# thomasjungblut/go-sstables

Hardware: AMD Instinct MI355X
Metric: recordio decode GiB/s (device-resident), v4 1 KiB records, 1/2/4/8 GPU (higher is better)
Workload: dtype u8; 1 GPU; C2: recordio v4, 1M x 1 KiB snappy records (text-like), one file per GPU; records=1000000, record_bytes=1024, decoded_bytes=1024000000, compression=snappy, parallelism=file-sharded x1 (1 files), no data-path collectives

## Files before the change

go-sstables_amd/csrc/rio_ctx.cpp:

```cpp
#include <algorithm>
#include <cstring>
#include <iterator>
#include <map>

#include "rio_ctx.h"
#include "rio_host.h"

using namespace rio;

extern "C" const char* rio_strerror(int s) {
    switch (s) {
    case RIO_OK: return "ok";
    case RIO_EOF: return "EOF";
    case RIO_EOF_ZERO_TAIL: return "EOF (zero-padded tail)";
    case RIO_EOF_HEADER: return "EOF inside record header";
    case RIO_EOF_PAYLOAD: return "EOF reading record payload";
    case RIO_ERR_UNEXPECTED_EOF: return "unexpected EOF";
    case RIO_ERR_MAGIC: return "magic number mismatch";
    case RIO_ERR_HEADER_CRC: return "header checksum mismatch";
    case RIO_ERR_VARINT_OVERFLOW: return "binary: varint overflows a 64-bit integer";
    case RIO_ERR_HEADER_TOO_LONG: return "checksum byte reader out of range";
    case RIO_ERR_DECOMPRESS: return "snappy: corrupt input";
    case RIO_ERR_VERSION: return "version mismatch";
    case RIO_ERR_COMPRESSION_TYPE: return "unknown compression type";
    case RIO_ERR_SHORT_FILE_HEADER: return "not enough bytes in the file header";
    case RIO_ERR_INVALID_OFFSET: return "mmap: invalid ReadAt offset";
    case RIO_ERR_UNSUPPORTED: return "not supported by the GPU decode path";
    case RIO_ERR_CAPACITY: return "output capacity too small";
    case RIO_ERR_ARG: return "invalid argument";
    case RIO_ERR_HIP: return "HIP runtime error";
    case RIO_ERR_STATE: return "reader state error";
    case RIO_ERR_IO: return "I/O error";
    case RIO_ERR_PROTO: return "proto: cannot parse invalid wire-format data";
    case RIO_EOF_CODEC: return "EOF from the codec (empty gzip payload)";
    default: return "unknown status";
    }
}

extern "C" int rio_status_is_eof(int s) {
    return s == RIO_EOF || s == RIO_EOF_ZERO_TAIL || s == RIO_EOF_HEADER || s == RIO_EOF_PAYLOAD || s == RIO_EOF_CODEC;
}

extern "C" const char* rio_build_info(void) { return "librio gfx950 recordio v3/v4 decode"; }

extern "C" uint64_t rio_max_records(uint64_t len) {
    return len <= RIO_FILE_HEADER_BYTES ? 1 : (len - RIO_FILE_HEADER_BYTES) / 5 + 1;
}

constexpr uint64_t kLaneWalkMin = 768, kLaneWalkMax = 8192, kLaneWalkChunks = 32768;
constexpr uint64_t kLaneWalkSmallMin = 512, kLaneWalkSmallChunks = 65536;
constexpr uint64_t kBigRecordChunk = 65536;
constexpr uint64_t kSmallFileChunkMin = 8192, kWalkWavesPerSimd = 5;
static uint64_t wave_chunk_bytes(const rio_ctx* ctx, uint64_t len) {
    const uint64_t cb = ctx->fr.chunk_bytes;
    if (!ctx->fr.chunk_auto) return cb;
    const uint64_t slots = ctx->fr.walk_slots;
    const uint64_t want = ((len + slots - 1) / slots + 4095) & ~4095ull;
    return std::min(cb, std::max(want, kSmallFileChunkMin));
}

struct ArenaSizes {
    uint64_t n_chunks, slots, n_blocks, scratch, meta;
};
static ArenaSizes arena_sizes(uint64_t len, uint64_t cb) {
    ArenaSizes z;
    z.n_chunks = len > RIO_FILE_HEADER_BYTES ? (len - RIO_FILE_HEADER_BYTES + cb - 1) / cb : 0;
    z.slots = cb / 5 + 1;
    z.n_blocks = (z.n_chunks + 255) / 256;
    const uint64_t nc = std::max<uint64_t>(z.n_chunks, 1), nb = std::max<uint64_t>(z.n_blocks, 1);
    z.scratch = nc * z.slots * 8;
    auto al = [](uint64_t x) { return (x + 255) & ~255ull; };
    z.meta = al(sizeof(ScanState)) + al(sizeof(rio_file_info)) + 2 * al(nb * sizeof(RunSum)) +
             al(2 * kFailLanes * sizeof(uint64_t)) + al(nc * sizeof(ChunkSum)) + al(nc * sizeof(RunSum)) +
             al(nc * sizeof(ChunkPlace));
    return z;
}

int rio::ctx_frame_params(rio_ctx* ctx, const uint8_t* d_file, uint64_t len, FrameParams& P, FileArenas& A,
                          bool reserve_all) {
    const rio_ctx::Framing& F = ctx->fr;
    memset(&P, 0, sizeof P);
    P.file = d_file;
    P.len = len;
    bool lane = F.walk_mode == 1;
    if (F.walk_mode == 2 && F.walk_hint && len / F.lane_chunk_bytes >= kLaneWalkChunks) {
        const uint64_t m = *reinterpret_cast<volatile uint64_t*>(F.walk_hint);
        const uint64_t chunks = len / F.lane_chunk_bytes;
        lane = (m >= kLaneWalkMin && m <= kLaneWalkMax) ||
               (m >= F.lane_walk_min && m < kLaneWalkMin && chunks >= kLaneWalkSmallChunks);
    }
    uint64_t cb = lane ? F.lane_chunk_bytes : wave_chunk_bytes(ctx, len);
    if (!lane && F.chunk_auto && F.walk_hint && *reinterpret_cast<volatile uint64_t*>(F.walk_hint) > kLaneWalkMax)
        cb = std::max<uint64_t>(cb, kBigRecordChunk);
    P.walk_lane = lane ? 1u : 0u;
    P.walk_hint = F.walk_hint;
    P.chunk_bytes = cb;
    P.coop_min = F.coop_min;
    P.comp_hint = RIO_COMP_UNKNOWN;
    P.zero_done = 0;
    const ArenaSizes z = arena_sizes(len, cb);
    P.n_chunks = z.n_chunks;
    P.slots = z.slots;
    P.n_blocks = z.n_blocks;
    const uint64_t nc = std::max<uint64_t>(P.n_chunks, 1), nb = std::max<uint64_t>(P.n_blocks, 1);
    uint64_t scr = z.scratch, meta_need = z.meta;
    if (reserve_all) {
        for (uint64_t c : {wave_chunk_bytes(ctx, len), F.chunk_bytes, F.lane_chunk_bytes,
                           std::max<uint64_t>(F.chunk_bytes, kBigRecordChunk)}) {
            const ArenaSizes y = arena_sizes(len, c);
            scr = std::max(scr, y.scratch);
            meta_need = std::max(meta_need, y.meta);
        }
    }
    HIP_TRY(A.scratch_off.ensure(scr));
    HIP_TRY(A.scratch_len.ensure(scr));
    HIP_TRY(A.scratch_pay.ensure(scr));
    auto al = [](uint64_t x) { return (x + 255) & ~255ull; };
    const uint64_t o_info = al(sizeof(ScanState)), o_brun = o_info + al(sizeof(rio_file_info));
    const uint64_t o_bexc = o_brun + al(nb * sizeof(RunSum)), o_fail = o_bexc + al(nb * sizeof(RunSum));
    const uint64_t o_chk = o_fail + al(2 * kFailLanes * sizeof(uint64_t)), o_cexc = o_chk + al(nc * sizeof(ChunkSum));
    const uint64_t o_place = o_cexc + al(nc * sizeof(RunSum)), meta_bytes = o_place + al(nc * sizeof(ChunkPlace));
    HIP_TRY(A.meta.ensure(std::max(meta_bytes, meta_need)));
    HIP_TRY(ctx->fr.sink.ensure(kSinkBytes));
    uint8_t* const mb = A.meta.as<uint8_t>();
    P.sink = F.sink.as<uint8_t>();
    P.fail_lanes = reinterpret_cast<uint64_t*>(mb + o_fail);
    P.scratch_off = A.scratch_off.as<uint64_t>();
    P.scratch_len = A.scratch_len.as<uint64_t>();
    P.scratch_pay = A.scratch_pay.as<uint64_t>();
    P.chunks = reinterpret_cast<ChunkSum*>(mb + o_chk);
    P.chunk_excl = reinterpret_cast<RunSum*>(mb + o_cexc);
    P.place = reinterpret_cast<ChunkPlace*>(mb + o_place);
    P.block_runs = reinterpret_cast<RunSum*>(mb + o_brun);
    P.block_excl = reinterpret_cast<RunSum*>(mb + o_bexc);
    P.state = reinterpret_cast<ScanState*>(mb);
    P.info = reinterpret_cast<rio_file_info*>(mb + o_info);
    return RIO_OK;
}

extern "C" int rio_device_count(int* out) {
    int n = 0;
    if (hipGetDeviceCount(&n) != hipSuccess) n = 0;
    if (out) *out = n;
    return n > 0 ? RIO_OK : RIO_ERR_HIP;
}

extern "C" int rio_ctx_create(int device, rio_ctx** out) {
    if (!out) return RIO_ERR_ARG;
    *out = nullptr;
    int n = 0;
    if (hipGetDeviceCount(&n) != hipSuccess || n <= 0) return RIO_ERR_HIP;
    if (device < 0 || device >= n) return RIO_ERR_ARG;
    HIP_TRY(hipSetDevice(device));
    auto* c = new rio_ctx();
    rio_ctx::Framing& F = c->fr;
    c->device = device;
    F.chunk_bytes = env_u64("RIO_CHUNK_BYTES", 32768);
    F.chunk_auto = std::getenv("RIO_CHUNK_BYTES") == nullptr;
    if (F.chunk_bytes < 64 || F.chunk_bytes > (1ull << 30) || (F.chunk_bytes & 15)) F.chunk_bytes = 32768;
    F.walk_mode = (uint32_t)std::min<uint64_t>(env_u64("RIO_WALK_LANE", 2), 2);
    F.lane_chunk_bytes = env_u64("RIO_LANE_CHUNK_BYTES", 16384);
    F.lane_walk_min = env_u64("RIO_LANE_WALK_MIN", kLaneWalkSmallMin);
    int cus = 0;
    if (hipDeviceGetAttribute(&cus, hipDeviceAttributeMultiprocessorCount, device) == hipSuccess && cus > 0)
        F.walk_slots = (uint64_t)cus * 4 * kWalkWavesPerSimd;
    if (F.lane_chunk_bytes < 64 || F.lane_chunk_bytes > (1ull << 30) || (F.lane_chunk_bytes & 15))
        F.lane_chunk_bytes = 16384;
    if (hipHostMalloc(reinterpret_cast<void**>(&F.walk_hint), sizeof(uint64_t), hipHostMallocPortable) != hipSuccess) {
        (void)hipGetLastError();
        F.walk_hint = nullptr;
    } else {
        *F.walk_hint = 0;
    }
    F.coop_min = env_u64("RIO_COOP_MIN", ~0ull >> 8);
    if (hipStreamCreateWithFlags(&c->stream, hipStreamNonBlocking) != hipSuccess) {
        delete c;
        return RIO_ERR_HIP;
    }
    c->timing.set_ring(0);
    *out = c;
    return RIO_OK;
}

extern "C" int rio_ctx_device(const rio_ctx* c) { return c ? c->device : -1; }

extern "C" void rio_ctx_destroy(rio_ctx* c) {
    if (!c) return;
    hipSetDevice(c->device);
    hipStreamSynchronize(c->stream);
    if (c->order.ev) hipEventSynchronize(c->order.ev);
    c->mrg.views.wait();
    c->wal.segs.wait();
    delete c;
}

extern "C" int rio_ctx_set_timing(rio_ctx* c, int slots) {
    if (!c || slots < 0) return RIO_ERR_ARG;
    hipSetDevice(c->device);
    hipStreamSynchronize(c->stream);
// ... 191 lines not shown
```

go-sstables_amd/csrc/rio_ctx.h:

```cpp
#pragma once
#include <hip/hip_runtime.h>

#include <algorithm>
#include <array>
#include <cstdlib>
#include <memory>
#include <mutex>
#include <vector>

#include "rio_host.h"
#include "rio_launch.h"

#define HIP_TRY(x)                                  \
    do {                                            \
        hipError_t e_ = (x);                        \
        if (e_ != hipSuccess) return RIO_ERR_HIP;   \
    } while (0)

namespace rio {

inline int hip_status(hipError_t e) { return e == hipSuccess ? RIO_OK : RIO_ERR_HIP; }

inline bool header_refused(int s) {
    return s == RIO_ERR_VERSION || s == RIO_ERR_COMPRESSION_TYPE || s == RIO_ERR_SHORT_FILE_HEADER;
// ... 1 lines not shown
inline bool nothing_framed(int s) { return header_refused(s) || s == RIO_ERR_UNSUPPORTED; }

inline uint64_t env_u64(const char* name, uint64_t dflt) {
    const char* v = getenv(name);
    if (!v || !*v) return dflt;
    return strtoull(v, nullptr, 0);
}

struct DevBuf {
    void* p = nullptr;
    size_t cap = 0;
    DevBuf() = default;
    DevBuf(const DevBuf&) = delete;
    DevBuf& operator=(const DevBuf&) = delete;
    ~DevBuf() { release(); }
    hipError_t ensure(size_t n) {
        if (n <= cap) return hipSuccess;
        release();
        size_t want = std::max<size_t>(n, 256);
        hipError_t e = hipMalloc(&p, want);
        if (e == hipSuccess) cap = want;
        return e;
    }
    void release() {
        if (p) hipFree(p);
        p = nullptr;
        cap = 0;
    }
    template <class T>
    T* as() const { return static_cast<T*>(p); }
};

struct FileArenas {
    DevBuf scratch_off, scratch_len, scratch_pay, rec_pay, rec_desc, meta;
    uint64_t bytes() const {
        return scratch_off.cap + scratch_len.cap + scratch_pay.cap + rec_pay.cap + rec_desc.cap + meta.cap;
    }
};

struct PlanUpload {
    DevBuf dev;
    std::vector<uint64_t> host;
    hipEvent_t ev = nullptr;
    ~PlanUpload() {
        wait();
        if (ev) hipEventDestroy(ev);
    }
    hipError_t upload(std::vector<uint64_t>& fresh, hipStream_t s) {
        hipError_t e = ev ? hipEventSynchronize(ev) : hipEventCreateWithFlags(&ev, hipEventDisableTiming);
        if (e != hipSuccess) return e;
        host.swap(fresh);
        e = hipMemcpyAsync(dev.p, host.data(), host.size() * 8, hipMemcpyHostToDevice, s);
        return e != hipSuccess ? e : hipEventRecord(ev, s);
    }
    void wait() const {
        if (ev) hipEventSynchronize(ev);
    }
};

}

struct rio_ctx {
    int device = 0;
    hipStream_t stream = nullptr;
    std::mutex mu;

    struct Timing {
        std::vector<std::array<hipEvent_t, 5>> ring;
        uint64_t cursor = 0;
// ... 144 lines not shown
```

go-sstables_amd/csrc/rio_device.h:

```cpp
#pragma once
#include <stdint.h>

#include "rio.h"

namespace rio {

constexpr uint64_t kNone = ~0ull;
constexpr uint64_t kNilBit = 1ull << 63;
constexpr uint64_t kBadBit = 1ull << 62;
constexpr uint64_t kEofBit = 1ull << 61;
constexpr uint64_t kLenMask = kEofBit - 1;
constexpr uint32_t kDescWide = 0xFFFFFFFFu;
constexpr uint32_t kFailLanes = 1024;

constexpr unsigned kSnappyBlock = 256;
#ifndef RIO_SNAPPY_GRID
#define RIO_SNAPPY_GRID 512
#endif
constexpr unsigned kSnappyGrid = RIO_SNAPPY_GRID;
constexpr unsigned kSnappyGridMax = 1024;
static_assert(kSnappyGrid <= kSnappyGridMax, "sink sized for kSnappyGridMax workgroups");
constexpr uint64_t kSinkBytes = (uint64_t)kSnappyBlock / 64 * kSnappyGridMax * 64;

struct ChunkSum {
    uint64_t entry;
    uint64_t exit;
    uint64_t bytes;
    uint64_t err_off;
    uint64_t det0, det1;
    uint32_t count;
    int32_t status;
};

struct RunSum {
    uint64_t key;
    uint64_t out;
    uint64_t cnt;
    uint64_t bytes;
    uint64_t ce;
    uint32_t term;
    uint32_t broken;
    uint64_t term_chunk;
};

struct ChunkPlace {
    uint64_t base_idx;
    uint64_t base_bytes;
    uint64_t owned;
};

struct ScanState {
    uint32_t version, compression;
    int32_t hdr_status;
    uint32_t slow;
    uint64_t n_records;
// ... 3 lines not shown
    uint64_t status_offset;
    uint64_t det0, det1;
    uint64_t zero_from;
    uint64_t n_repairs;
    uint64_t first_bad;
    uint64_t n_bad;
    uint64_t unsupported_rec;
    uint32_t n_fail_lanes;
    uint32_t capacity_fail;
    uint32_t huge_streams;
    uint32_t any_mixed;
    uint32_t scan_ticket;
    uint32_t finish_ticket;
    uint32_t pipe_next;
    uint32_t gz_resize;
    uint32_t gz_redo;
};

struct ReadAtResult {
    int32_t status;
    int32_t nil;
    uint64_t len;
    uint64_t det0, det1;
    uint64_t hdr_len;
    uint64_t payload_off;
};

struct FrameParams {
    const uint8_t* file;
    uint64_t len;
    uint64_t chunk_bytes;
    uint64_t n_chunks;
    uint64_t slots;
    uint64_t* scratch_off;
    uint64_t* scratch_len;
    uint64_t* scratch_pay;
    uint64_t* rec_pay;
    uint4* rec_desc;
    uint8_t* sink;
    uint64_t* fail_lanes;
    uint64_t coop_min;
    uint32_t comp_hint;
    uint32_t zero_done;
    uint32_t walk_lane;
    uint64_t* walk_hint;
    uint32_t redo;
    ChunkSum* chunks;
    RunSum* block_runs;
    RunSum* chunk_excl;
    ChunkPlace* place;
    uint64_t* block_in;
    RunSum* block_excl;
    uint64_t n_blocks;
    ScanState* state;
    uint8_t* out;
    uint64_t out_cap;
    uint64_t* out_off;
    uint64_t* rec_off;
    uint8_t* flags;
    uint64_t rec_cap;
    rio_file_info* info;
};

constexpr uint32_t kMaxBatch = 16;
struct FrameBatch {
    FrameParams f[kMaxBatch];
    uint32_t n;
};

// ... 160 lines not shown
    const uint64_t* src;
    const uint8_t* keep;
    uint64_t* order;
    uint64_t* pfx;
    uint64_t* n_sel;
    uint64_t* result;
};
struct MemLookupParams {
    rio_mem_index i0, i1;
    uint32_t n_idx;
    const uint8_t* keys;
    const uint64_t* key_off;
    uint64_t n;
    uint64_t key_bytes;
    uint64_t* src;
};
struct DbParams {
    rio_mem_index i0, i1;
    uint32_t n_idx;
    const rio_sst_view* views;
    const uint64_t* const* stored;
    uint32_t T;
    uint32_t check_crc;
    const uint64_t* tab_src;
    const uint64_t* mem_src;
    uint64_t n;
    uint8_t* status;
    uint64_t* tmp;
    uint64_t* val_off;
    uint8_t* values;
    uint64_t values_cap;
};

#ifdef __HIPCC__
#define RIO_HD __host__ __device__
#else
#define RIO_HD
#endif
RIO_HD inline uint32_t pb_varint_len(uint64_t v) {
    uint32_t n = 1;
    while (v >= 0x80) {
        v >>= 7;
        n++;
    }
    return n;
}
RIO_HD inline uint64_t pb_index_entry_len(uint64_t key_len, uint64_t value_off, uint64_t checksum) {
    return (key_len ? 1 + pb_varint_len(key_len) + key_len : 0) + (value_off ? 1 + pb_varint_len(value_off) : 0) +
           (checksum ? 1 + pb_varint_len(checksum) : 0);
}

#ifdef __HIPCC__
__device__ inline void mark_bad(const FrameParams& P, uint64_t i, uint8_t flag = RIO_FLAG_CORRUPT) {
    P.flags[i] = (uint8_t)(P.flags[i] | flag);
    atomicMin((unsigned long long*)&P.state->first_bad, (unsigned long long)i);
    atomicAdd((unsigned long long*)&P.state->n_bad, 1ull);
}
__device__ inline void rec_stream(const FrameParams& P, uint64_t i, uint64_t& start, uint64_t& slen) {
    const uint4 d = P.rec_desc[i];
    if (d.z == kDescWide && d.w == kDescWide) {
        const uint64_t pay = P.rec_pay[i];
        start = P.rec_off[i] + (pay & 0xFF);
        slen = pay >> 8;
    } else {
        start = ((uint64_t)d.y << 32) | d.x;
        slen = d.z;
    }
}
#endif

}
// ... 1 lines not shown
```

go-sstables_amd/csrc/rio_gzip.hip:

```cpp
#include <hip/hip_runtime.h>

#include "rio_device.h"
#include "rio_dev_util.h"
#include "rio_launch.h"

namespace rio {

namespace {
constexpr uint32_t kGzWaves = 4;
constexpr uint32_t kGzIn = 2048;
constexpr uint32_t kGzTinyIn = 1024;
constexpr uint32_t kGzTinyWin = 1024;
constexpr uint32_t kGzSmallWin = 2048;
constexpr uint32_t kGzLargeWin = 32768;
constexpr uint32_t kFastBits = 9;
constexpr uint32_t kFastSize = 1u << kFastBits;
#ifndef RIO_GZ_RUN
#define RIO_GZ_RUN 1
#endif
constexpr uint64_t kPayFail = 1ull << 63;
constexpr uint64_t kPayResize = 1ull << 62;
constexpr uint64_t kPayLen = ~(kPayFail | kPayResize);
__constant__ uint8_t kClenOrder[19] = {16, 17, 18, 0, 8, 7, 9, 6, 10, 5, 11, 4, 12, 3, 13, 2, 14, 1, 15};

// ... 666 lines not shown
        const uint8_t* t = P.file + P.rec_off[i] + (pay & 0xFF) + slen - 8;
        const uint32_t want = t[0] | (uint32_t)t[1] << 8 | (uint32_t)t[2] << 16 | (uint32_t)t[3] << 24;
        const uint8_t* o = P.out + P.out_off[i];
        const uint64_t len = P.out_off[i + 1] - P.out_off[i];
        uint32_t c = 0xFFFFFFFFu;
        uint64_t k = 0;
        for (; k < len && ((uintptr_t)(o + k) & 15u); k++) c = tab[(c ^ o[k]) & 0xFFu] ^ (c >> 8);
        for (; k + 16 <= len; k += 16) {
            const uint4 v = *reinterpret_cast<const uint4*>(o + k);
            const uint32_t w[4] = {v.x, v.y, v.z, v.w};
#pragma unroll
            for (int j = 0; j < 16; j++) c = tab[(c ^ (w[j >> 2] >> (8 * (j & 3)))) & 0xFFu] ^ (c >> 8);
        }
        for (; k < len; k++) c = tab[(c ^ o[k]) & 0xFFu] ^ (c >> 8);
        if ((c ^ 0xFFFFFFFFu) != want) mark_bad(P, i);
    }
}

__global__ void __launch_bounds__(64 * kGzWaves) k_gz_resize(FrameParams P) {
    extern __shared__ __attribute__((aligned(16))) uint8_t lds[];
    ScanState* st = P.state;
    if (!st->gz_resize || !gzip_active(P, st)) return;
    const uint32_t lane = threadIdx.x & 63u, wv = threadIdx.x >> 6;
    if (!st->slow && blockIdx.x == 0 && threadIdx.x == 0) {
        st->gz_redo = 1u;
        st->scan_ticket = 0;
        st->first_bad = kNone;
        st->n_bad = 0;
    }
    using Lds = GzLds<kGzLargeWin, kGzIn>;
    Lds& S = *reinterpret_cast<Lds*>(lds + wv * sizeof(Lds));
    for (uint64_t c = (uint64_t)blockIdx.x * kGzWaves + wv; c < P.n_chunks; c += (uint64_t)gridDim.x * kGzWaves) {
    const ChunkPlace pl = P.place[c];
    uint64_t* sl = P.scratch_len + c * P.slots;
    for (uint64_t k = 0; k < pl.owned; k++) {
        const uint64_t i = pl.base_idx + k;
        const uint64_t pay = P.rec_pay[i];
        if (!(pay & kPayResize)) continue;
        if (st->slow) {
            if (lane == 0) atomicMin((unsigned long long*)&st->unsupported_rec, (unsigned long long)i);
            continue;
        }
        uint64_t total = 0;
        const int rc = gz_record<kGzLargeWin, kGzIn, true>(S, P.file + P.rec_off[i] + (pay & 0xFF),
                                                              (uint32_t)((pay & kPayLen) >> 8), nullptr, 0, lane, &total);
        if (lane == 0) {
            if (rc == kGzOk) {
                const uint64_t old = sl[k] & kLenMask;
                sl[k] = (sl[k] & ~kLenMask) | total;
                P.chunks[c].bytes += total - old;
            } else if (rc == kGzCorrupt) {
                sl[k] |= kBadBit;
            } else {
                atomicMin((unsigned long long*)&st->unsupported_rec, (unsigned long long)i);
            }
        }
    }
    }
}

hipError_t launch_gzip_resize(const FrameParams& P, hipStream_t s) {
    hipLaunchKernelGGL(k_gz_resize, dim3(256), dim3(64 * kGzWaves), kGzWaves * sizeof(GzLds<kGzLargeWin, kGzIn>),
                       s, P);
    return hipGetLastError();
}

hipError_t launch_gzip_decode(const FrameParams& P, hipStream_t s) {
    hipLaunchKernelGGL(k_gzip_inflate<kGzTinyWin>, dim3(gz_grid<kGzTinyWin>()), dim3(64 * gz_waves<kGzTinyWin>()),
                       gz_lds_bytes<kGzTinyWin>(), s, P);
    hipLaunchKernelGGL(k_gzip_inflate<kGzSmallWin>, dim3(gz_grid<kGzSmallWin>()), dim3(64 * kGzWaves),
                       gz_lds_bytes<kGzSmallWin>(), s, P);
    hipLaunchKernelGGL(k_gzip_inflate<kGzLargeWin>, dim3(gz_grid<kGzLargeWin>()), dim3(64 * kGzWaves),
                       gz_lds_bytes<kGzLargeWin>(), s, P);
    hipLaunchKernelGGL(k_gzip_crc, dim3(512), dim3(256), 0, s, P);
    return hipGetLastError();
}

}
```

go-sstables_amd/csrc/rio_kernels.hip:

```cpp
#include <hip/hip_ext.h>
#include <hip/hip_runtime.h>

#include <vector>

#include "rio_device.h"
#include "rio_dev_util.h"
#include "rio_launch.h"
#include "rio_pb.h"

namespace rio {

#ifndef RIO_SCAN_PROBE
#define RIO_SCAN_PROBE 0
#endif
#if RIO_SCAN_PROBE
__device__ unsigned long long g_probe[32];
#define PROBE_MIN(i) atomicMin(&g_probe[i], (unsigned long long)wall_clock64())
#define PROBE_MAX(i) atomicMax(&g_probe[i], (unsigned long long)wall_clock64())
#else
#define PROBE_MIN(i) ((void)0)
#define PROBE_MAX(i) ((void)0)
#endif

__device__ __forceinline__ uint32_t code_pf(uint32_t lines) {
// ... 388 lines not shown
}
__device__ __forceinline__ uint64_t chunk_end(const FrameParams& P, uint64_t c) {
    uint64_t e = chunk_start(P, c) + P.chunk_bytes;
    return e < P.len ? e : P.len;
}

__device__ __forceinline__ uint32_t magic3(uint32_t ver) { return ver == RIO_VERSION1 ? 0x130691u : 0x4C8D91u; }

__device__ uint64_t find_entry(const FrameParams& P, uint64_t cs, uint64_t ce, uint32_t ver, uint32_t comp) {
    const uint8_t* f = P.file;
    const uint32_t m3 = magic3(ver);
    for (uint64_t q = cs & ~15ull; q < ce; q += 16) {
        const uint4 w = *reinterpret_cast<const uint4*>(f + q);
        uint32_t ws[4] = {w.x, w.y, w.z, w.w};
#pragma unroll
        for (int k = 0; k < 4; k++) {
            uint32_t x = ws[k] ^ 0x91919191u;
            uint32_t hit = (x - 0x01010101u) & ~x & 0x80808080u;
            while (hit) {
                int b = __builtin_ctz(hit) >> 3;
                hit &= hit - 1;
                uint64_t p = q + 4 * k + b;
                if (p < cs || p >= ce || p + 2 >= P.len) continue;
                if (f[p + 1] != ((m3 >> 8) & 0xFF) || f[p + 2] != (m3 >> 16)) continue;
                Hdr h;
                uint64_t nx, ol, pd, lf;
                if (frame_record(f, P.len, p, ver, comp, h, nx, ol, pd, lf) == RIO_OK) return p;
            }
        }
    }
    return kNone;
}

__device__ void walk_from(const FrameParams& P, uint64_t c, uint64_t p, uint32_t ver, uint32_t comp, ChunkSum& s,
                          const uint32_t* crct = nullptr) {
    const uint64_t ce = chunk_end(P, c);
    uint64_t* so = P.scratch_off + c * P.slots;
    uint64_t* sl = P.scratch_len + c * P.slots;
    uint64_t* sp = P.scratch_pay + c * P.slots;
    while (p < ce) {
        Hdr h;
        uint64_t next = 0, olen = 0, pd = 0, lf = 0;
        int e = frame_record(P.file, P.len, p, ver, comp, h, next, olen, pd, lf, crct);
        if (e) {
            s.status = e;
            s.err_off = p;
            if (e == RIO_ERR_HEADER_CRC) {
                s.det0 = h.exp_crc;
                s.det1 = h.act_crc;
            } else if (e == RIO_ERR_MAGIC) {
                s.det0 = h.magic_len;
            } else if (e == RIO_ERR_UNEXPECTED_EOF && h.hdr_len != 0) {
                s.det0 = 1;
            }
            break;
        }
        if (s.count < P.slots) {
            so[s.count] = p;
            sl[s.count] = olen | lf | (h.nil ? kNilBit : 0);
            sp[s.count] = pd;
        }
        s.count++;
        s.bytes += olen;
        p = next;
    }
    s.exit = s.status ? s.err_off : p;
}

__device__ __forceinline__ ChunkSum chunk_sum_empty(uint64_t entry) {
    ChunkSum s;
    s.entry = entry;
    s.exit = kNone;
    s.bytes = 0;
    s.err_off = 0;
    s.det0 = s.det1 = 0;
    s.count = 0;
    s.status = RIO_OK;
    return s;
}

__device__ void walk_chunk(const FrameParams& P, uint64_t c, uint64_t from, uint32_t ver, uint32_t comp) {
    ChunkSum s = chunk_sum_empty(from);
    if (from != kNone) walk_from(P, c, from, ver, comp, s);
    P.chunks[c] = s;
}

template <typename T>
__device__ __forceinline__ T wave_excl_scan(T v, uint32_t lane) {
    T x = v;
#pragma unroll
    for (uint32_t d = 1; d < 64; d <<= 1) {
        const T y = __shfl_up(x, d);
        if (lane >= d) x += y;
    }
// ... 107 lines not shown
}

#ifndef RIO_COPY_GRID
#define RIO_COPY_GRID 4096
#endif
#ifndef RIO_COPY_SMALL
#define RIO_COPY_SMALL 128
#endif
constexpr uint64_t kCopySmall = RIO_COPY_SMALL;
#ifndef RIO_WALK_OCC
#define RIO_WALK_OCC 5
#endif
#if RIO_SCAN_PROBE
__device__ unsigned long long g_wave[1 << 18][6];
#endif
#if RIO_WALK_OCC
__global__ void __launch_bounds__(64 * kWalkWaves, RIO_WALK_OCC) k_walk(FrameParams P) {
#else
__global__ void __launch_bounds__(64 * kWalkWaves) k_walk(FrameParams P) {
#endif
    __shared__ WalkLds W[kWalkWaves];
    __shared__ uint32_t crct[1024];
    const uint32_t pf = code_pf(blockIdx.x < kPfBlocks ? kPfWalk : 0);
    if (threadIdx.x == 0) PROBE_MIN(0);
    if (blockIdx.x == 0 && threadIdx.x == 0) init_state(P);
    crc32c_tab_init(crct);
    const uint32_t lane = threadIdx.x & 63u, wv = threadIdx.x >> 6;
    const uint64_t c = (uint64_t)blockIdx.x * kWalkWaves + wv;
    uint32_t ver, comp;
    if (c >= P.n_chunks || file_header_status(P, ver, comp) != RIO_OK) return;
    WalkLds& L = W[wv];
    const uint64_t cs = chunk_start(P, c), ce = chunk_end(P, c);
    const uint8_t* f = P.file;
    uint64_t* so = P.scratch_off + c * P.slots;
    uint64_t* sl = P.scratch_len + c * P.slots;
    uint64_t* sp = P.scratch_pay + c * P.slots;
    uint64_t p = (c == 0) ? (uint64_t)RIO_FILE_HEADER_BYTES : kNone;
    uint32_t mode = (c == 0) ? 1u : 0u;
    uint64_t count = 0, bytes = 0, entry = p;
    uint64_t ws = cs;
#if RIO_SCAN_PROBE
    const unsigned long long tw0 = wall_clock64();
    unsigned long long tfill = 0, tframe = 0, nwin = 0, nround = 0, tq = 0;
#endif
    while (ws < ce && mode < 2) {
        if (mode == 1) {
            if (p >= ce) break;
            ws = umax(ws, p);
        }
#if RIO_SCAN_PROBE
        tq = wall_clock64();
        nwin++;
#endif
        if (lane == 0) L.overflow = kNone;
        uint32_t total = 0;
        uint64_t rd = ws & ~15ull;
        uint32_t added = 1;
        for (uint32_t r = 0; r < kWalkFillMax && rd < ce && total < kWalkFill && total <= 64 && (total == 0 || added);
             r++) {
            uint4 blk[4];
            uint32_t tail[4];
#pragma unroll
            for (uint32_t j = 0; j < 4; j++) {
                const uint64_t q = rd + 1024 * j + 16 * lane;
                if (q < ce) {
                    blk[j] = *reinterpret_cast<const uint4*>(f + q);
                    tail[j] = *reinterpret_cast<const uint32_t*>(f + q + 16);
                }
            }
// ... 60 lines not shown
#if RIO_SCAN_PROBE
        {
            const unsigned long long t = wall_clock64();
            tframe += t - tq;
            tq = t;
        }
#endif
        const uint64_t succ_pos = __shfl_down(cpos, 1);
        if (mode == 0) {
            const uint32_t k = lane_ffs(ok_mask);
            if (k < 64) {
                p = readlane64(cpos, k);
                mode = 1;
            }
            entry = p;
        }
        uint32_t slot = ~0u;
        while (mode == 1 && p < we) {
            const uint32_t e0 = lane_ffs(__ballot(have && cpos >= p));
            if (e0 >= nst || readlane64(cpos, e0) != p || !((ok_mask >> e0) & 1)) {
                mode = 2;
                break;
            }
            const bool link = ok && lane + 1 < nst && nx == succ_pos;
            const uint64_t brk = ~__ballot(link) & (~0ull << e0);
            const uint32_t b = lane_ffs(brk);
            const bool bok = (ok_mask >> b) & 1;
            const uint32_t last = bok ? b : b - 1;
            if (lane >= e0 && lane <= last) slot = (uint32_t)count + (lane - e0);
            count += last - e0 + 1;
            p = bok ? readlane64(nx, b) : readlane64(cpos, b);
        }
        const uint64_t mylen = slot != ~0u ? ol : 0;
        if (slot != ~0u && slot < P.slots) {
            so[slot] = cpos;
            sl[slot] = ol | lf | (h.nil ? kNilBit : 0);
            sp[slot] = pd;
        }
        uint64_t wsum;
        wave_excl_scan64(mylen, lane, wsum);
        bytes += wsum;
        wave_sync_lds();
        ws = we;
    }
    if (lane == 0) {
        ChunkSum s = chunk_sum_empty(entry);
        s.count = (uint32_t)count;
        s.bytes = bytes;
        if (mode == 2)
            walk_from(P, c, p, ver, comp, s);
        else if (entry != kNone)
            s.exit = p;
        P.chunks[c] = s;
        PROBE_MAX(1);
#if RIO_SCAN_PROBE
        if (c < (1u << 18)) {
            const unsigned long long te = wall_clock64();
            g_wave[c][0] = tw0;
            g_wave[c][1] = te;
            g_wave[c][2] = tfill;
            g_wave[c][3] = tframe;
            g_wave[c][4] = nwin;
            g_wave[c][5] = nround;
        }
#endif
    }
    code_pf_done(pf);
}

__device__ uint64_t find_entry_lane(const FrameParams& P, uint64_t cs, uint64_t ce, uint32_t ver, uint32_t comp,
                                    const uint32_t* crct) {
// ... 20 lines not shown
#pragma unroll
        for (uint32_t j = 0; j < 8; j++) {
            const uint32_t nx = j < 7 ? a[j + 1].x : t;
            const uint32_t d[5] = {a[j].x, a[j].y, a[j].z, a[j].w, nx};
            const uint64_t m = (uint64_t)magic_mask(d, q0 + 16 * j, cs, ce, P.len, m3) << (16 * (j & 3));
            if (j < 4)
                mlo |= m;
            else
                mhi |= m;
        }
        while (mlo | mhi) {
            const bool lo = mlo != 0;
            const uint64_t mm = lo ? mlo : mhi;
            const uint64_t p = q0 + (lo ? 0u : 64u) + (uint64_t)__builtin_ctzll(mm);
            if (lo)
                mlo &= mlo - 1;
            else
                mhi &= mhi - 1;
            Hdr hd;
            uint64_t nxp, ol, pd, lf;
            if (frame_record(f, P.len, p, ver, comp, hd, nxp, ol, pd, lf, crct) == RIO_OK) return p;
        }
        if (q1 >= ce) return kNone;
        q0 = q1;
#pragma unroll
        for (uint32_t j = 0; j < 8; j++) a[j] = na[j];
        t = nt;
    }
}

__device__ void walk_from_lane(const FrameParams& P, uint64_t c, uint64_t p, uint32_t ver, uint32_t comp, ChunkSum& s,
                               const uint32_t* crct) {
    const uint8_t* f = P.file;
    const uint64_t ce = chunk_end(P, c);
    uint64_t* so = P.scratch_off + c * P.slots;
    uint64_t* sl = P.scratch_len + c * P.slots;
    uint64_t* sp = P.scratch_pay + c * P.slots;
    bool have = p < ce && p + 32 <= P.len;
    uint4 a = zero4(), b = zero4();
    if (have) {
        a = ldu16(f + p);
        b = ldu16(f + p + 16);
    }
    while (p < ce) {
        Hdr h;
        uint64_t next = 0, olen = 0, pd = 0, lf = 0;
        int e = kFrameSlow;
        if (have) {
            const uint32_t w[8] = {a.x, a.y, a.z, a.w, b.x, b.y, b.z, b.w};
            e = frame_fast(w, P.len, p, ver, comp, h, next, olen, pd, crct);
        }
        if (e != RIO_OK) e = frame_slow(f, P.len, p, ver, comp, h, next, olen, pd, lf);
        if (e) {
            s.status = e;
            s.err_off = p;
            if (e == RIO_ERR_HEADER_CRC) {
                s.det0 = h.exp_crc;
                s.det1 = h.act_crc;
            } else if (e == RIO_ERR_MAGIC) {
                s.det0 = h.magic_len;
            } else if (e == RIO_ERR_UNEXPECTED_EOF && h.hdr_len != 0) {
                s.det0 = 1;
            }
            break;
        }
        have = next < ce && next + 32 <= P.len;
        if (have) {
            a = ldu16(f + next);
            b = ldu16(f + next + 16);
        }
        if (s.count < P.slots) {
            so[s.count] = p;
            sl[s.count] = olen | lf | (h.nil ? kNilBit : 0);
            sp[s.count] = pd;
        }
        s.count++;
        s.bytes += olen;
        p = next;
    }
    s.exit = s.status ? s.err_off : p;
}

constexpr uint32_t kWalkLaneBlock = 256;
#if RIO_SCAN_PROBE
__device__ unsigned long long g_lane[1 << 18][4];
#endif
__global__ void __launch_bounds__(kWalkLaneBlock) k_walk_lane(FrameParams P) {
    __shared__ uint32_t crct[1024];
#if RIO_SCAN_PROBE
    const unsigned long long ta = wall_clock64();
#endif
    if (blockIdx.x == 0 && threadIdx.x == 0) init_state(P);
    crc32c_tab_init(crct);
    const uint64_t c = (uint64_t)blockIdx.x * kWalkLaneBlock + threadIdx.x;
    uint32_t ver, comp;
    if (c >= P.n_chunks || file_header_status(P, ver, comp) != RIO_OK) return;
    const uint64_t cs = chunk_start(P, c), ce = chunk_end(P, c);
#if RIO_SCAN_PROBE
    const unsigned long long tb = wall_clock64();
#endif
    const uint64_t from = c == 0 ? (uint64_t)RIO_FILE_HEADER_BYTES : find_entry_lane(P, cs, ce, ver, comp, crct);
#if RIO_SCAN_PROBE
    const unsigned long long tc = wall_clock64();
#endif
    ChunkSum s = chunk_sum_empty(from);
    if (from != kNone) walk_from_lane(P, c, from, ver, comp, s, crct);
    P.chunks[c] = s;
#if RIO_SCAN_PROBE
// ... 268 lines not shown
    const uint32_t tag = p[0];
    if (tag & 3u) return 0;
    const uint32_t x = tag >> 2;
    uint64_t L;
    uint32_t h;
    if (x < 60) {
        L = (uint64_t)x + 1;
        h = 1;
    } else {
        const uint32_t nb = x - 59;
        if (slen < 1 + nb) return 0;
        uint64_t v = 0;
        for (uint32_t b = 0; b < nb; b++) v |= (uint64_t)p[1 + b] << (8 * b);
        L = v + 1;
        h = 1 + nb;
    }
    return (L == len && h + L == slen) ? h : 0u;
}
__device__ __forceinline__ bool snappy_single_literal(const uint8_t* p, uint64_t slen, uint64_t len) {
    return snappy_literal_hdr(p, slen, len) != 0;
}

struct PlaceFlags {
    uint64_t first_bad;
    uint64_t n_bad;
    bool mixed;
    bool huge;
};

template <uint32_t G>
__device__ PlaceFlags place_chunk(const FrameParams& P, uint64_t c, uint64_t base_idx, uint64_t base_bytes,
                                  uint64_t owned, bool snappy, bool pay_all, uint32_t lane) {
    PlaceFlags fl{kNone, 0, false, false};
    const uint64_t* so = P.scratch_off + c * P.slots;
    const uint64_t* sl = P.scratch_len + c * P.slots;
    const uint64_t* sp = P.scratch_pay + c * P.slots;
    bool mixed = false, huge = false;
    uint64_t carry = base_bytes;
    uint64_t l_n = 0, ro_n = 0, pay_n = 0;
    if (lane < owned) {
        l_n = sl[lane];
        ro_n = so[lane];
        pay_n = sp[lane];
    }
    for (uint64_t k0 = 0; k0 < owned; k0 += G) {
        const uint64_t k = k0 + lane;
        const bool v = k < owned;
        const uint64_t l = l_n, ro = ro_n, pay = pay_n, len = v ? l & kLenMask : 0;
        if (k + G < owned) {
            l_n = sl[k + G];
            ro_n = so[k + G];
            pay_n = sp[k + G];
        }
        uint64_t wsum;
        const uint64_t excl = G == 64 ? wave_excl_scan64(len, lane, wsum) : group16_excl_scan64(len, lane, wsum);
        bool bad = false;
        if (v) {
            const uint64_t i = base_idx + k;
            const uint64_t start = ro + (pay & 0xFF), slen = pay >> 8;
            const bool wide = slen >= kDescWide || len >= kDescWide;
            P.rec_off[i] = ro;
            if (pay_all || wide) P.rec_pay[i] = pay;
            P.out_off[i] = carry + excl;
            const uint8_t fg = ((l & kNilBit) ? RIO_FLAG_NIL : 0) | ((l & kBadBit) ? RIO_FLAG_CORRUPT : 0) |
                               ((l & kEofBit) ? RIO_FLAG_EOF : 0);
            P.flags[i] = fg;
            bad = (fg & (RIO_FLAG_CORRUPT | RIO_FLAG_EOF)) != 0;
            P.rec_desc[i] = make_uint4((uint32_t)start, (uint32_t)(start >> 32), wide ? kDescWide : (uint32_t)slen,
                                       wide ? kDescWide : (uint32_t)len);
            huge = huge || wide;
            if (snappy && fg == 0) mixed |= !snappy_single_literal(P.file + start, slen, len);
        }
        const uint64_t bm = group_ballot<G>(bad);
        if (bm) {
            fl.n_bad += (uint64_t)__popcll(bm);
            if (fl.first_bad == kNone) fl.first_bad = base_idx + k0 + (uint64_t)__builtin_ctzll(bm);
        }
        carry += wsum;
        snappy = snappy && !group_ballot<G>(mixed);
        mixed = mixed || !snappy;
    }
    fl.mixed = group_ballot<G>(mixed) != 0;
    fl.huge = group_ballot<G>(huge) != 0;
    return fl;
}
// ... 919 lines not shown
```

go-sstables_amd/csrc/rio_lzw.hip:

```cpp
#include <hip/hip_runtime.h>

#include <type_traits>

#include "rio_device.h"
#include "rio_dev_util.h"
#include "rio_launch.h"

namespace rio {

namespace {
constexpr uint32_t kLzMaxK = 3840;
constexpr uint32_t kLzSmallK = 1024, kLzSmallLen = kLzSmallK * 9 / 8;
constexpr uint32_t kLzSmallGrid = 256 * 32;
constexpr uint64_t kLzResize = 1ull << 62;
constexpr uint64_t kLzLen = ~(3ull << 62);
constexpr uint32_t kLzGrid = 1536;
enum : uint32_t { kLit = 0, kCopy = 1, kClear = 2, kEnd = 3, kBad = 4, kMissing = 5 };
enum : int { kLzOk = 0, kLzResize_ = 1, kLzCorrupt = 2, kLzUnsupported = 3 };

template <uint32_t kMaxK>
using LzPos = typename std::conditional<kMaxK == 1024, uint16_t, uint32_t>::type;
template <uint32_t kMaxK>
struct LzLds {
    LzPos<kMaxK> pos[kMaxK];
// ... 169 lines not shown
        const uint64_t pay = P.rec_pay[i];
        const uint64_t slen = (pay & kLzLen) >> 8;
        if ((slen <= kLzSmallLen && dlen < 65536) != kSmall) continue;
        if (slen >= 0xFFFFFFF0ull || dlen >= 0xFFFFFFF0ull) {
            if (lane == 0) atomicMin((unsigned long long*)&st->unsupported_rec, (unsigned long long)i);
            continue;
        }
        const int rc = lz_record<false, kMaxK>(S, P.file + P.rec_off[i] + (pay & 0xFF), (uint32_t)slen, P.out + o0,
                                        (uint32_t)dlen, lane, nullptr);
        if (lane == 0) {
            if (rc == kLzResize_ && !P.redo) {
                P.rec_pay[i] = pay | kLzResize;
                st->gz_resize = 1u;
            } else if (rc != kLzOk) {
                mark_bad(P, i);
            }
        }
    }
}

__global__ void __launch_bounds__(64) k_lzw_resize(FrameParams P) {
    __shared__ LzLds<kLzMaxK> S;
    ScanState* st = P.state;
    if (!st->gz_resize || !lzw_active(P, st)) return;
    const uint32_t lane = threadIdx.x;
    if (!st->slow && blockIdx.x == 0 && lane == 0) {
        st->gz_redo = 1u;
        st->scan_ticket = 0;
        st->first_bad = kNone;
        st->n_bad = 0;
    }
    for (uint64_t c = blockIdx.x; c < P.n_chunks; c += gridDim.x) {
        const ChunkPlace pl = P.place[c];
        uint64_t* sl = P.scratch_len + c * P.slots;
        for (uint64_t k = 0; k < pl.owned; k++) {
            const uint64_t i = pl.base_idx + k;
            const uint64_t pay = P.rec_pay[i];
            if (!(pay & kLzResize)) continue;
            if (st->slow) {
                if (lane == 0) atomicMin((unsigned long long*)&st->unsupported_rec, (unsigned long long)i);
                continue;
            }
            uint64_t total = 0;
            const int rc = lz_record<true, kLzMaxK>(S, P.file + P.rec_off[i] + (pay & 0xFF), (uint32_t)((pay & kLzLen) >> 8),
                                           nullptr, 0, lane, &total);
            if (lane == 0) {
                if (rc == kLzOk && total < 0xFFFFFFF0ull) {
                    const uint64_t old = sl[k] & kLenMask;
                    sl[k] = (sl[k] & ~kLenMask) | total;
                    P.chunks[c].bytes += total - old;
                } else if (rc == kLzCorrupt) {
                    sl[k] |= kBadBit;
                } else {
                    atomicMin((unsigned long long*)&st->unsupported_rec, (unsigned long long)i);
                }
            }
        }
    }
}

hipError_t launch_lzw_decode(const FrameParams& P, hipStream_t s) {
    hipLaunchKernelGGL(k_lzw_decode<kLzSmallK>, dim3(kLzSmallGrid), dim3(64), 0, s, P);
    hipLaunchKernelGGL(k_lzw_decode<kLzMaxK>, dim3(kLzGrid), dim3(64), 0, s, P);
    return hipGetLastError();
}

hipError_t launch_lzw_resize(const FrameParams& P, hipStream_t s) {
    hipLaunchKernelGGL(k_lzw_resize, dim3(kLzGrid), dim3(64), 0, s, P);
    return hipGetLastError();
}

}
```

Before: 472.4 GiB/s.

## Pack walk scratch into one 16-byte slot per record

Replaces the three separate 8-byte scratch arrays (offset, length, payload) written by the record walkers and read by place_chunk with a single 16-byte WalkSlot. The offset becomes chunk-relative and is packed together with the header size and stream length in one 64-bit word. Each slot is then written and read with one 128-bit access, which cuts scratch memory traffic from 24 to 16 bytes per record and uses fewer, wider transactions. Stream lengths too large for the packed field are escaped and recomputed from the next record's offset, which adds a branch and an extra load in that rare case. A lane-walk threshold constant is also lowered, so the lane walker is selected for smaller files.

```diff
diff --git a/go-sstables_amd/csrc/rio_ctx.cpp b/go-sstables_amd/csrc/rio_ctx.cpp
--- a/go-sstables_amd/csrc/rio_ctx.cpp
+++ b/go-sstables_amd/csrc/rio_ctx.cpp
@@ -48,7 +48,7 @@
 }
 
 constexpr uint64_t kLaneWalkMin = 768, kLaneWalkMax = 8192, kLaneWalkChunks = 32768;
-constexpr uint64_t kLaneWalkSmallMin = 512, kLaneWalkSmallChunks = 65536;
+constexpr uint64_t kLaneWalkSmallMin = 512, kLaneWalkSmallChunks = 32768;
 constexpr uint64_t kBigRecordChunk = 65536;
 constexpr uint64_t kSmallFileChunkMin = 8192, kWalkWavesPerSimd = 5;
 static uint64_t wave_chunk_bytes(const rio_ctx* ctx, uint64_t len) {
@@ -68,7 +68,7 @@
     z.slots = cb / 5 + 1;
     z.n_blocks = (z.n_chunks + 255) / 256;
     const uint64_t nc = std::max<uint64_t>(z.n_chunks, 1), nb = std::max<uint64_t>(z.n_blocks, 1);
-    z.scratch = nc * z.slots * 8;
+    z.scratch = nc * z.slots * sizeof(WalkSlot);
     auto al = [](uint64_t x) { return (x + 255) & ~255ull; };
     z.meta = al(sizeof(ScanState)) + al(sizeof(rio_file_info)) + 2 * al(nb * sizeof(RunSum)) +
              al(2 * kFailLanes * sizeof(uint64_t)) + al(nc * sizeof(ChunkSum)) + al(nc * sizeof(RunSum)) +
@@ -112,9 +112,7 @@
             meta_need = std::max(meta_need, y.meta);
         }
     }
-    HIP_TRY(A.scratch_off.ensure(scr));
-    HIP_TRY(A.scratch_len.ensure(scr));
-    HIP_TRY(A.scratch_pay.ensure(scr));
+    HIP_TRY(A.scratch.ensure(scr));
     auto al = [](uint64_t x) { return (x + 255) & ~255ull; };
     const uint64_t o_info = al(sizeof(ScanState)), o_brun = o_info + al(sizeof(rio_file_info));
     const uint64_t o_bexc = o_brun + al(nb * sizeof(RunSum)), o_fail = o_bexc + al(nb * sizeof(RunSum));
@@ -125,9 +123,7 @@
     uint8_t* const mb = A.meta.as<uint8_t>();
     P.sink = F.sink.as<uint8_t>();
     P.fail_lanes = reinterpret_cast<uint64_t*>(mb + o_fail);
-    P.scratch_off = A.scratch_off.as<uint64_t>();
-    P.scratch_len = A.scratch_len.as<uint64_t>();
-    P.scratch_pay = A.scratch_pay.as<uint64_t>();
+    P.scratch = A.scratch.as<WalkSlot>();
     P.chunks = reinterpret_cast<ChunkSum*>(mb + o_chk);
     P.chunk_excl = reinterpret_cast<RunSum*>(mb + o_cexc);
     P.place = reinterpret_cast<ChunkPlace*>(mb + o_place);
@@ -157,14 +153,16 @@
     c->device = device;
     F.chunk_bytes = env_u64("RIO_CHUNK_BYTES", 32768);
     F.chunk_auto = std::getenv("RIO_CHUNK_BYTES") == nullptr;
-    if (F.chunk_bytes < 64 || F.chunk_bytes > (1ull << 30) || (F.chunk_bytes & 15)) F.chunk_bytes = 32768;
+    static_assert(kMaxChunkBytes == 1ull << 30 && kMaxChunkBytes <= 1ull << kSlotOffBits,
+                  "the chunk cap bounds WalkSlot's chunk-relative offsets and k_walk's 32-bit differences");
+    if (F.chunk_bytes < 64 || F.chunk_bytes > kMaxChunkBytes || (F.chunk_bytes & 15)) F.chunk_bytes = 32768;
     F.walk_mode = (uint32_t)std::min<uint64_t>(env_u64("RIO_WALK_LANE", 2), 2);
     F.lane_chunk_bytes = env_u64("RIO_LANE_CHUNK_BYTES", 16384);
     F.lane_walk_min = env_u64("RIO_LANE_WALK_MIN", kLaneWalkSmallMin);
     int cus = 0;
     if (hipDeviceGetAttribute(&cus, hipDeviceAttributeMultiprocessorCount, device) == hipSuccess && cus > 0)
         F.walk_slots = (uint64_t)cus * 4 * kWalkWavesPerSimd;
-    if (F.lane_chunk_bytes < 64 || F.lane_chunk_bytes > (1ull << 30) || (F.lane_chunk_bytes & 15))
+    if (F.lane_chunk_bytes < 64 || F.lane_chunk_bytes > kMaxChunkBytes || (F.lane_chunk_bytes & 15))
         F.lane_chunk_bytes = 16384;
     if (hipHostMalloc(reinterpret_cast<void**>(&F.walk_hint), sizeof(uint64_t), hipHostMallocPortable) != hipSuccess) {
         (void)hipGetLastError();
diff --git a/go-sstables_amd/csrc/rio_ctx.h b/go-sstables_amd/csrc/rio_ctx.h
--- a/go-sstables_amd/csrc/rio_ctx.h
+++ b/go-sstables_amd/csrc/rio_ctx.h
@@ -57,9 +57,9 @@
 };
 
 struct FileArenas {
-    DevBuf scratch_off, scratch_len, scratch_pay, rec_pay, rec_desc, meta;
+    DevBuf scratch, rec_pay, rec_desc, meta;
     uint64_t bytes() const {
-        return scratch_off.cap + scratch_len.cap + scratch_pay.cap + rec_pay.cap + rec_desc.cap + meta.cap;
+        return scratch.cap + rec_pay.cap + rec_desc.cap + meta.cap;
     }
 };
 
diff --git a/go-sstables_amd/csrc/rio_device.h b/go-sstables_amd/csrc/rio_device.h
--- a/go-sstables_amd/csrc/rio_device.h
+++ b/go-sstables_amd/csrc/rio_device.h
@@ -4,6 +4,12 @@
 #include "rio.h"
 
 namespace rio {
+
+#ifdef __HIPCC__
+#define RIO_HD __host__ __device__
+#else
+#define RIO_HD
+#endif
 
 constexpr uint64_t kNone = ~0ull;
 constexpr uint64_t kNilBit = 1ull << 63;
@@ -21,6 +27,23 @@
 constexpr unsigned kSnappyGridMax = 1024;
 static_assert(kSnappyGrid <= kSnappyGridMax, "sink sized for kSnappyGridMax workgroups");
 constexpr uint64_t kSinkBytes = (uint64_t)kSnappyBlock / 64 * kSnappyGridMax * 64;
+
+constexpr uint64_t kMaxChunkBytes = 1ull << 30;
+
+struct alignas(16) WalkSlot {
+    uint64_t len;
+    uint64_t pos;
+};
+constexpr uint32_t kSlotOffBits = 30, kSlotHdrShift = 30, kSlotStreamShift = 39;
+constexpr uint64_t kSlotEsc = 1ull << 38;
+constexpr uint64_t kSlotStreamEsc = 1ull << (64 - kSlotStreamShift);
+RIO_HD inline WalkSlot slot_pack(uint64_t rel, uint64_t len_flags, uint64_t pay) {
+    const uint64_t slen = pay >> 8;
+    return WalkSlot{len_flags, rel | (pay & 0xFF) << kSlotHdrShift |
+                                   (slen < kSlotStreamEsc ? slen << kSlotStreamShift : kSlotEsc)};
+}
+RIO_HD inline uint64_t slot_rel(uint64_t pos) { return pos & ((1ull << kSlotOffBits) - 1); }
+RIO_HD inline uint64_t slot_pay(uint64_t pos) { return (pos >> kSlotStreamShift) << 8 | ((pos >> kSlotHdrShift) & 0xFF); }
 
 struct ChunkSum {
     uint64_t entry;
@@ -90,9 +113,7 @@
     uint64_t chunk_bytes;
     uint64_t n_chunks;
     uint64_t slots;
-    uint64_t* scratch_off;
-    uint64_t* scratch_len;
-    uint64_t* scratch_pay;
+    WalkSlot* scratch;
     uint64_t* rec_pay;
     uint4* rec_desc;
     uint8_t* sink;
@@ -319,11 +340,6 @@
     uint64_t values_cap;
 };
 
-#ifdef __HIPCC__
-#define RIO_HD __host__ __device__
-#else
-#define RIO_HD
-#endif
 RIO_HD inline uint32_t pb_varint_len(uint64_t v) {
     uint32_t n = 1;
     while (v >= 0x80) {
diff --git a/go-sstables_amd/csrc/rio_gzip.hip b/go-sstables_amd/csrc/rio_gzip.hip
--- a/go-sstables_amd/csrc/rio_gzip.hip
+++ b/go-sstables_amd/csrc/rio_gzip.hip
@@ -722,7 +722,7 @@
     Lds& S = *reinterpret_cast<Lds*>(lds + wv * sizeof(Lds));
     for (uint64_t c = (uint64_t)blockIdx.x * kGzWaves + wv; c < P.n_chunks; c += (uint64_t)gridDim.x * kGzWaves) {
     const ChunkPlace pl = P.place[c];
-    uint64_t* sl = P.scratch_len + c * P.slots;
+    WalkSlot* sc = P.scratch + c * P.slots;
     for (uint64_t k = 0; k < pl.owned; k++) {
         const uint64_t i = pl.base_idx + k;
         const uint64_t pay = P.rec_pay[i];
@@ -736,11 +736,11 @@
                                                               (uint32_t)((pay & kPayLen) >> 8), nullptr, 0, lane, &total);
         if (lane == 0) {
             if (rc == kGzOk) {
-                const uint64_t old = sl[k] & kLenMask;
-                sl[k] = (sl[k] & ~kLenMask) | total;
+                const uint64_t old = sc[k].len & kLenMask;
+                sc[k].len = (sc[k].len & ~kLenMask) | total;
                 P.chunks[c].bytes += total - old;
             } else if (rc == kGzCorrupt) {
-                sl[k] |= kBadBit;
+                sc[k].len |= kBadBit;
             } else {
                 atomicMin((unsigned long long*)&st->unsupported_rec, (unsigned long long)i);
             }
diff --git a/go-sstables_amd/csrc/rio_kernels.hip b/go-sstables_amd/csrc/rio_kernels.hip
--- a/go-sstables_amd/csrc/rio_kernels.hip
+++ b/go-sstables_amd/csrc/rio_kernels.hip
@@ -444,12 +444,20 @@
     return kNone;
 }
 
+__device__ __forceinline__ void slot_store(WalkSlot* s, uint64_t rel, uint64_t len_flags, uint64_t pay) {
+    const WalkSlot v = slot_pack(rel, len_flags, pay);
+    *reinterpret_cast<uint4*>(s) =
+        make_uint4((uint32_t)v.len, (uint32_t)(v.len >> 32), (uint32_t)v.pos, (uint32_t)(v.pos >> 32));
+}
+__device__ __forceinline__ WalkSlot slot_load(const WalkSlot* s) {
+    const uint4 v = *reinterpret_cast<const uint4*>(s);
+    return WalkSlot{(uint64_t)v.y << 32 | v.x, (uint64_t)v.w << 32 | v.z};
+}
+
 __device__ void walk_from(const FrameParams& P, uint64_t c, uint64_t p, uint32_t ver, uint32_t comp, ChunkSum& s,
                           const uint32_t* crct = nullptr) {
-    const uint64_t ce = chunk_end(P, c);
-    uint64_t* so = P.scratch_off + c * P.slots;
-    uint64_t* sl = P.scratch_len + c * P.slots;
-    uint64_t* sp = P.scratch_pay + c * P.slots;
+    const uint64_t cs = chunk_start(P, c), ce = chunk_end(P, c);
+    WalkSlot* sc = P.scratch + c * P.slots;
     while (p < ce) {
         Hdr h;
         uint64_t next = 0, olen = 0, pd = 0, lf = 0;
@@ -467,11 +475,7 @@
             }
             break;
         }
-        if (s.count < P.slots) {
-            so[s.count] = p;
-            sl[s.count] = olen | lf | (h.nil ? kNilBit : 0);
-            sp[s.count] = pd;
-        }
+        if (s.count < P.slots) slot_store(sc + s.count, p - cs, olen | lf | (h.nil ? kNilBit : 0), pd);
         s.count++;
         s.bytes += olen;
         p = next;
@@ -645,9 +649,7 @@
     WalkLds& L = W[wv];
     const uint64_t cs = chunk_start(P, c), ce = chunk_end(P, c);
     const uint8_t* f = P.file;
-    uint64_t* so = P.scratch_off + c * P.slots;
-    uint64_t* sl = P.scratch_len + c * P.slots;
-    uint64_t* sp = P.scratch_pay + c * P.slots;
+    WalkSlot* sc = P.scratch + c * P.slots;
     uint64_t p = (c == 0) ? (uint64_t)RIO_FILE_HEADER_BYTES : kNone;
     uint32_t mode = (c == 0) ? 1u : 0u;
     uint64_t count = 0, bytes = 0, entry = p;
@@ -774,11 +776,7 @@
             p = bok ? readlane64(nx, b) : readlane64(cpos, b);
         }
         const uint64_t mylen = slot != ~0u ? ol : 0;
-        if (slot != ~0u && slot < P.slots) {
-            so[slot] = cpos;
-            sl[slot] = ol | lf | (h.nil ? kNilBit : 0);
-            sp[slot] = pd;
-        }
+        if (slot != ~0u && slot < P.slots) slot_store(sc + slot, cpos - cs, ol | lf | (h.nil ? kNilBit : 0), pd);
         uint64_t wsum;
         wave_excl_scan64(mylen, lane, wsum);
         bytes += wsum;
@@ -865,10 +863,8 @@
 __device__ void walk_from_lane(const FrameParams& P, uint64_t c, uint64_t p, uint32_t ver, uint32_t comp, ChunkSum& s,
                                const uint32_t* crct) {
     const uint8_t* f = P.file;
-    const uint64_t ce = chunk_end(P, c);
-    uint64_t* so = P.scratch_off + c * P.slots;
-    uint64_t* sl = P.scratch_len + c * P.slots;
-    uint64_t* sp = P.scratch_pay + c * P.slots;
+    const uint64_t cs = chunk_start(P, c), ce = chunk_end(P, c);
+    WalkSlot* sc = P.scratch + c * P.slots;
     bool have = p < ce && p + 32 <= P.len;
     uint4 a = zero4(), b = zero4();
     if (have) {
@@ -902,11 +898,7 @@
             a = ldu16(f + next);
             b = ldu16(f + next + 16);
         }
-        if (s.count < P.slots) {
-            so[s.count] = p;
-            sl[s.count] = olen | lf | (h.nil ? kNilBit : 0);
-            sp[s.count] = pd;
-        }
+        if (s.count < P.slots) slot_store(sc + s.count, p - cs, olen | lf | (h.nil ? kNilBit : 0), pd);
         s.count++;
         s.bytes += olen;
         p = next;
@@ -1241,25 +1233,22 @@
 __device__ PlaceFlags place_chunk(const FrameParams& P, uint64_t c, uint64_t base_idx, uint64_t base_bytes,
                                   uint64_t owned, bool snappy, bool pay_all, uint32_t lane) {
     PlaceFlags fl{kNone, 0, false, false};
-    const uint64_t* so = P.scratch_off + c * P.slots;
-    const uint64_t* sl = P.scratch_len + c * P.slots;
-    const uint64_t* sp = P.scratch_pay + c * P.slots;
+    const uint64_t cs = chunk_start(P, c);
+    const WalkSlot* sc = P.scratch + c * P.slots;
     bool mixed = false, huge = false;
     uint64_t carry = base_bytes;
-    uint64_t l_n = 0, ro_n = 0, pay_n = 0;
-    if (lane < owned) {
-        l_n = sl[lane];
-        ro_n = so[lane];
-        pay_n = sp[lane];
-    }
+    WalkSlot s_n{0, 0};
+    if (lane < owned) s_n = slot_load(sc + lane);
     for (uint64_t k0 = 0; k0 < owned; k0 += G) {
         const uint64_t k = k0 + lane;
         const bool v = k < owned;
-        const uint64_t l = l_n, ro = ro_n, pay = pay_n, len = v ? l & kLenMask : 0;
-        if (k + G < owned) {
-            l_n = sl[k + G];
-            ro_n = so[k + G];
-            pay_n = sp[k + G];
+        const uint64_t l = s_n.len, ro = cs + slot_rel(s_n.pos), len = v ? l & kLenMask : 0;
+        uint64_t pay = slot_pay(s_n.pos);
+        const bool esc = v && (s_n.pos & kSlotEsc);
+        if (k + G < owned) s_n = slot_load(sc + k + G);
+        if (esc) {
+            const uint64_t nx = k + 1 < owned ? cs + slot_rel(sc[k + 1].pos) : P.chunks[c].exit;
+            pay |= (nx - ro - pay) << 8;
         }
         uint64_t wsum;
         const uint64_t excl = G == 64 ? wave_excl_scan64(len, lane, wsum) : group16_excl_scan64(len, lane, wsum);
diff --git a/go-sstables_amd/csrc/rio_lzw.hip b/go-sstables_amd/csrc/rio_lzw.hip
--- a/go-sstables_amd/csrc/rio_lzw.hip
+++ b/go-sstables_amd/csrc/rio_lzw.hip
@@ -225,7 +225,7 @@
     }
     for (uint64_t c = blockIdx.x; c < P.n_chunks; c += gridDim.x) {
         const ChunkPlace pl = P.place[c];
-        uint64_t* sl = P.scratch_len + c * P.slots;
+        WalkSlot* sc = P.scratch + c * P.slots;
         for (uint64_t k = 0; k < pl.owned; k++) {
             const uint64_t i = pl.base_idx + k;
             const uint64_t pay = P.rec_pay[i];
@@ -239,11 +239,11 @@
                                            nullptr, 0, lane, &total);
             if (lane == 0) {
                 if (rc == kLzOk && total < 0xFFFFFFF0ull) {
-                    const uint64_t old = sl[k] & kLenMask;
-                    sl[k] = (sl[k] & ~kLenMask) | total;
+                    const uint64_t old = sc[k].len & kLenMask;
+                    sc[k].len = (sc[k].len & ~kLenMask) | total;
                     P.chunks[c].bytes += total - old;
                 } else if (rc == kLzCorrupt) {
-                    sl[k] |= kBadBit;
+                    sc[k].len |= kBadBit;
                 } else {
                     atomicMin((unsigned long long*)&st->unsupported_rec, (unsigned long long)i);
                 }
```

Measured after the change: 477.8 GiB/s (median of 6 runs). 1.01x the previous value.
